# Socrates666/esp32-wake-word

Hardware: AMD Instinct MI355X
Metric: audio windows/sec (1s@16kHz, 40-MFCC) through xiaoa CNN at 1/2/4/8 MI355X (higher is better)
Workload: dtype f32; 1 GPU; config2: fused MFCC(torchaudio+CMVN)+xiaoa CNN fp32, B clips per GPU; audio=fp32 samples, batch_per_gpu=65536, global_batch=65536, seq_len=16000, parallelism=dp1 (per-rank clip split, no collectives), process_group_world_size=1

## Files before the change

### esp32-wake-word_amd/csrc/wk_fe_dev.h

```cpp
#pragma once
#include "wk_common.h"
#include "wk_tables.h"

namespace wk {

__device__ __forceinline__ f2 w32(int k2) {
  switch (k2) {
    case 0: return {1.0f, 0.0f};
    case 1: return {0.98078528040323043f, -0.19509032201612825f};
    case 2: return {0.92387953251128674f, -0.38268343236508978f};
    case 3: return {0.83146961230254524f, -0.55557023301960218f};
    case 4: return {0.70710678118654752f, -0.70710678118654752f};
    case 5: return {0.55557023301960218f, -0.83146961230254524f};
    case 6: return {0.38268343236508978f, -0.92387953251128674f};
    case 7: return {0.19509032201612825f, -0.98078528040323043f};
    default: return {0.0f, -1.0f};
  }
}

template <typename T>
struct Raw {
  T x0[10], x1[10];
  T xb;
};

template <typename T> __device__ __forceinline__ T raw_ld(__amdgpu_buffer_rsrc_t r, int idx);
template <> __device__ __forceinline__ float raw_ld<float>(__amdgpu_buffer_rsrc_t r, int idx) {
  return __builtin_bit_cast(float, __builtin_amdgcn_raw_buffer_load_b32(r, idx * 4, 0, 0));
}
template <> __device__ __forceinline__ int16_t raw_ld<int16_t>(__amdgpu_buffer_rsrc_t r, int idx) {
  return (int16_t)__builtin_amdgcn_raw_buffer_load_b16(r, idx * 2, 0, 0);
}

template <typename T> __device__ __forceinline__ void raw_ld2(__amdgpu_buffer_rsrc_t r, int idx, T& a, T& b);
template <> __device__ __forceinline__ void raw_ld2<float>(__amdgpu_buffer_rsrc_t r, int idx, float& a, float& b) {
  const auto v = __builtin_amdgcn_raw_buffer_load_b64(r, idx * 4, 0, 0);
  a = __uint_as_float(v[0]);
  b = __uint_as_float(v[1]);
}
template <> __device__ __forceinline__ void raw_ld2<int16_t>(__amdgpu_buffer_rsrc_t r, int idx, int16_t& a,
                                                            int16_t& b) {
  const uint32_t v = __builtin_amdgcn_raw_buffer_load_b32(r, idx * 2, 0, 0);
  a = (int16_t)(v & 0xFFFFu);
  b = (int16_t)(v >> 16);
}

__device__ __forceinline__ int refl_idx(int i, int n) {
  i = i < 0 ? -i : i;
  return i > n - 1 ? 2 * (n - 1) - i : i;
}

template <bool MODE_B, typename T>
__device__ __forceinline__ void load_raw(__amdgpu_buffer_rsrc_t rs, int base, int j, int n, bool act, bool general,
                                         Raw<T>& r, int off = 0) {
  if (!act) return;
  if (!general) {
    const int v0 = base + 2 * j;
#pragma unroll
    for (int n1 = 0; n1 < 10; ++n1) raw_ld2<T>(rs, v0 + 32 * n1, r.x0[n1], r.x1[n1]);
    r.xb = raw_ld<T>(rs, base - 1);
  } else {
#pragma unroll
    for (int n1 = 0; n1 < 10; ++n1) {
      const int i0 = base + 32 * n1 + 2 * j;
      r.x0[n1] = raw_ld<T>(rs, off + (MODE_B ? refl_idx(i0, n) : i0));
      r.x1[n1] = raw_ld<T>(rs, off + (MODE_B ? refl_idx(i0 + 1, n) : i0 + 1));
    }
    const int ib = j == 15 ? base + 32 * 9 + 32 : base - 1;
    r.xb = raw_ld<T>(rs, off + (MODE_B ? refl_idx(ib, n) : ib));
  }
}

__device__ __forceinline__ constexpr int pf_part(int n1) {
  return WK_FE_STAGED ? n1 / 3 : (n1 < 4 ? 0 : n1 < 7 ? 1 : n1 < 9 ? 2 : 3);
}
template <bool MODE_B, typename T>
__device__ __forceinline__ void load_raw_part(__amdgpu_buffer_rsrc_t rs, int base, int j, int n, bool act,
                                              bool general, Raw<T>& r, int part) {
  if (!act) return;
  if (general) {
    if (part == 0) load_raw<MODE_B, T>(rs, base, j, n, act, true, r);
    return;
  }
  const int v0 = base + 2 * j;
#pragma unroll
  for (int n1 = 0; n1 < 10; ++n1)
    if (pf_part(n1) == part) raw_ld2<T>(rs, v0 + 32 * n1, r.x0[n1], r.x1[n1]);
  if (part == 0) r.xb = raw_ld<T>(rs, base - 1);
}

struct NoPrefetch {
  __device__ __forceinline__ void operator()(int) const {}
};

__device__ __forceinline__ float row_ror1(float v) {
  return __int_as_float(__builtin_amdgcn_mov_dpp(__float_as_int(v), 0x121, 0xF, 0xF, false));
}
__device__ __forceinline__ float row_rol1(float v) {
  return __int_as_float(__builtin_amdgcn_mov_dpp(__float_as_int(v), 0x12F, 0xF, 0xF, false));
}

struct FeTables {
  const float* win;
  const float* tw;
};

struct TwsLds {
  const float* p;
  __device__ __forceinline__ f2 operator()(int k2, int j) const {
    return *reinterpret_cast<const f2*>(p + ((k2 - 1) * 16 + j) * 2);
  }
};

__device__ __forceinline__ bool fe_split_flip(int j, int k2) {
  return j == 8 || (j >= 1 && j <= 7 && !(k2 & 1)) || (j >= 9 && (k2 & 1));
}
__device__ __forceinline__ f2 fe_split_tw(int j, int k2) {
  float sn, cs;
  sincospif(-(float)(j + 16 * k2) / 256.0f, &sn, &cs);
  return fe_split_flip(j, k2) ? f2{-cs, sn} : f2{cs, sn};
}
__device__ __forceinline__ void fe_init_tws(float* tws, int tid, int nthreads) {
  for (int i = tid; i < 7 * 16; i += nthreads) {
    const f2 w = fe_split_tw(i % 16, i / 16 + 1);
    tws[2 * i] = w.x;
    tws[2 * i + 1] = w.y;
  }
}

template <bool MODE_B, typename T>
__device__ __forceinline__ void fe_stage0(const Raw<T>& raw, int base, int n, int j, bool general,
                                          const FeTables& tb, f2 (&a)[16], float pre = -0.97f WK_SP_PARAM) {
  f2 w[10];
#pragma unroll
  for (int n1 = 0; n1 < 10; ++n1) w[n1] = *reinterpret_cast<const f2*>(tb.win + 32 * n1 + 2 * j);
  float prev_rot = 0.0f;
  float y0[10], y1[10];
#pragma unroll
  for (int n1 = 0; n1 < 10; ++n1) {
    const float x0 = to_f(raw.x0[n1]), x1 = to_f(raw.x1[n1]);
    float rot = row_ror1(x1);
    asm volatile("" : "+v"(rot));
    const float xm = j != 0 ? rot : (n1 == 0 ? to_f(raw.xb) : prev_rot);
    prev_rot = rot;
    y0[n1] = __builtin_fmaf(pre, xm, x0);
    y1[n1] = __builtin_fmaf(pre, x0, x1);
  }
  if (MODE_B && general) {
#pragma unroll
    for (int n1 = 0; n1 < 10; ++n1) {
      const float x0 = to_f(raw.x0[n1]), x1 = to_f(raw.x1[n1]);
      const int i0 = base + 32 * n1 + 2 * j;
      float nx = row_rol1(x0);
      float nx1 = row_rol1(to_f(raw.x0[n1 + 1 < 10 ? n1 + 1 : 9]));
      asm volatile("" : "+v"(nx), "+v"(nx1));
      const float xn = j != 15 ? nx : (n1 < 9 ? nx1 : to_f(raw.xb));
      const bool reflected = i0 < 0 || i0 > n - 1;
      const float r0 = __builtin_fmaf(pre, x1, x0), r1 = __builtin_fmaf(pre, xn, x1);
      const float g0 = reflected ? r0 : (i0 == 0 ? x0 : y0[n1]);
      const float g1 = reflected ? r1 : y1[n1];
      a[n1] = f2{g0, g1} * w[n1];
    }
  } else {
#pragma unroll
    for (int n1 = 0; n1 < 10; ++n1) a[n1] = f2{y0[n1], y1[n1]} * w[n1];
  }
#pragma unroll
  for (int n1 = 10; n1 < 16; ++n1) a[n1] = f2{0.0f, 0.0f};
}

template <bool MODE_B, typename PF, typename TWS>
__device__ __forceinline__ void fe_rest(f2 (&a)[16], int j, float* __restrict__ row, float* __restrict__ xs,
                                        const FeTables& tb, f2 w0, const TWS& tws, int esp_pack,
                                        const PF& pf WK_SP_PARAM) {
  pf(0);
  dft16(a);
  WK_FE_HIT(2);

  f2* x2 = reinterpret_cast<f2*>(xs);
  const int wb = 17 * (j & 7) + (j & 8);
  auto tw = [&](int s) { return cmul2(a[dft16_out(s)], *reinterpret_cast<const f2*>(tb.tw + (s * 16 + j) * 2)); };
  f2 b[8];
  if constexpr (!WK_FE_STAGED) pf(1);
#pragma unroll
  for (int s = 0; s < 8; ++s) b[s] = tw(s);
  pf(-1);
#pragma unroll
  for (int s = 0; s < 8; ++s) x2[wb + s] = b[s];
  WK_FE_HIT(3);
  if constexpr (WK_FE_STAGED) pf(1);
  f2 c[16];
  wave_lds_sync();
#pragma unroll
  for (int s = 0; s < 8; ++s) c[s] = x2[j + 17 * s];
  if constexpr (!WK_FE_STAGED) pf(2);
#pragma unroll
  for (int s = 8; s < 16; ++s) b[s - 8] = tw(s);
  wave_lds_sync();
#pragma unroll
  for (int s = 8; s < 16; ++s) x2[wb + s - 8] = b[s - 8];
  wave_lds_sync();
#pragma unroll
  for (int s = 8; s < 16; ++s) c[s] = x2[(j ^ 8) + 17 * (s - 8)];
  wave_lds_sync();
  WK_FE_HIT(4);

  if constexpr (WK_FE_STAGED) {
    pf(2);
    dft16(c);
    pf(3);
  } else {
    pf(3);
    dft16(c);
  }
  WK_FE_HIT(5);

  f2 sc0 = {1.0f, 1.0f}, sc = {1.0f, 1.0f};
  if constexpr (!MODE_B) {
    const float e = esp_pack ? 4.0f / 2048.0f : 1.0f / 2048.0f;
    sc = f2{e, e};
    sc0 = esp_pack ? (j == 0 ? f2{1.0f / 2048.0f, 0.0f} : sc) : sc;
  }
  {
    const f2 z = c[dft16_out(8)];
    float p128 = 4.0f * __builtin_fmaf(z.x, z.x, z.y * z.y);
    if constexpr (!MODE_B) p128 = __builtin_fmaf(p128, sc.x, 1e-12f);
    if (j == 0) row[128] = p128;
  }
  constexpr int G = 3;
#pragma unroll
  for (int k0 = 0; k0 < 8; k0 += G) {
    f2 S[G], D[G], pw[G];
#if WK_FE_STAGED
    float mx[G], my[G];
#pragma unroll
    for (int t = 0; t < G; ++t)
      if (k0 + t <= 7) {
        const f2 sv = c[dft16_out(15 - k0 - t)];
        mx[t] = dpp<0x140>(sv.x);
        my[t] = dpp<0x140>(sv.y);
      }
#pragma unroll
    for (int t = 0; t < G; ++t) {
      const int k2 = k0 + t;
      if (k2 > 7) continue;
      const f2 zk = c[dft16_out(k2)];
      const f2 own = c[dft16_out((16 - k2) & 15)];
      f2 zq;
      zq.x = __int_as_float(__builtin_amdgcn_update_dpp(__float_as_int(own.x), __float_as_int(mx[t]), 0x111, 0xF, 0xF, false));
      zq.y = __int_as_float(__builtin_amdgcn_update_dpp(__float_as_int(own.y), __float_as_int(my[t]), 0x111, 0xF, 0xF, false));
      S[t] = fma2(zq, f2{1.0f, -1.0f}, zk);
      D[t] = fma2(zq, f2{-1.0f, 1.0f}, zk);
    }
#else
#pragma unroll
    for (int t = 0; t < G; ++t) {
      const int k2 = k0 + t;
      if (k2 > 7) continue;
      const f2 zk = c[dft16_out(k2)];
      const f2 sv = c[dft16_out(15 - k2)];
      const f2 own = c[dft16_out((16 - k2) & 15)];
      f2 zq;
      zq.x = __int_as_float(__builtin_amdgcn_update_dpp(__float_as_int(own.x), __float_as_int(dpp<0x140>(sv.x)),
                                                        0x111, 0xF, 0xF, false));
      zq.y = __int_as_float(__builtin_amdgcn_update_dpp(__float_as_int(own.y), __float_as_int(dpp<0x140>(sv.y)),
                                                        0x111, 0xF, 0xF, false));
      S[t] = fma2(zq, f2{1.0f, -1.0f}, zk);
      D[t] = fma2(zq, f2{-1.0f, 1.0f}, zk);
    }
#endif
#if WK_FE_STAGED
    f2 wt[G], tt[G], bb[G], uvx[G], uvy[G], sq[G];
#pragma unroll
    for (int t = 0; t < G; ++t)
      if (k0 + t <= 7) {
        wt[t] = k0 + t == 0 ? w0 : tws(k0 + t, j);
        tt[t] = cmul2_a(D[t], wt[t]);
      }
#pragma unroll
    for (int t = 0; t < G; ++t)
      if (k0 + t <= 7) bb[t] = cmul2_b(D[t], wt[t], tt[t]);
#pragma unroll
    for (int t = 0; t < G; ++t)
      if (k0 + t <= 7) {
        uvx[t] = fma2(by(bb[t]), f2{1.0f, -1.0f}, bx(S[t]));
        uvy[t] = fma2(bx(bb[t]), f2{-1.0f, 1.0f}, by(S[t]));
      }
#pragma unroll
    for (int t = 0; t < G; ++t)
      if (k0 + t <= 7) sq[t] = uvy[t] * uvy[t];
#pragma unroll
    for (int t = 0; t < G; ++t) {
      const int k2 = k0 + t;
      if (k2 > 7) continue;
      pw[t] = fma2(uvx[t], uvx[t], sq[t]);
      if constexpr (!MODE_B) pw[t] = fma2(pw[t], k2 == 0 ? sc0 : sc, f2{1e-12f, 1e-12f});
    }
#else
#pragma unroll
    for (int t = 0; t < G; ++t) {
      const int k2 = k0 + t;
      if (k2 > 7) continue;
      const f2 bb = cmul2(D[t], k2 == 0 ? w0 : tws(k2, j));
      const f2 uvx = fma2(by(bb), f2{1.0f, -1.0f}, bx(S[t]));
      const f2 uvy = fma2(bx(bb), f2{-1.0f, 1.0f}, by(S[t]));
      pw[t] = fma2(uvx, uvx, uvy * uvy);
      if constexpr (!MODE_B) pw[t] = fma2(pw[t], k2 == 0 ? sc0 : sc, f2{1e-12f, 1e-12f});
    }
#endif
#pragma unroll
    for (int t = 0; t < G; ++t)
      if (k0 + t <= 7) row[j + 16 * (k0 + t)] = pw[t].x;
#pragma unroll
    for (int t = 0; t < G; ++t)
      if (k0 + t <= 7) row[256 - j - 16 * (k0 + t)] = pw[t].y;
  }
  WK_FE_HIT(6);
}

template <bool MODE_B, int W>
__device__ __forceinline__ void mel_wave(const float* p, float* l) {
  if constexpr (MODE_B) melB_wave<W>(p, l); else melA_wave<W>(p, l);
}

template <bool MODE_B>
__device__ __forceinline__ void mel_dispatch(int wave, const float* p, float* l) {
  switch (wave) {
    case 0: mel_wave<MODE_B, 0>(p, l); break;
    case 1: mel_wave<MODE_B, 1>(p, l); break;
    case 2: mel_wave<MODE_B, 2>(p, l); break;
    case 3: mel_wave<MODE_B, 3>(p, l); break;
    case 4: mel_wave<MODE_B, 4>(p, l); break;
    case 5: mel_wave<MODE_B, 5>(p, l); break;
    case 6: mel_wave<MODE_B, 6>(p, l); break;
    default: mel_wave<MODE_B, 7>(p, l); break;
  }
}

__device__ __forceinline__ float cmvn_lane(float v, bool valid, int n) {
  const float mean = wave_sum(valid ? v : 0.0f) / (float)n;
  const float d = valid ? v - mean : 0.0f;
  float sd = sqrtf(wave_sum(d * d) / (float)(n - 1));
  sd = sd == 0.0f ? 1.0f : sd;
  return d * (1.0f / (sd + 1e-8f));
}

__device__ __forceinline__ void cmvn_lane2(float& v0, float& v1, bool valid, int n) {
  const float m0 = wave_sum(valid ? v0 : 0.0f) / (float)n;
  const float m1 = wave_sum(valid ? v1 : 0.0f) / (float)n;
  const float d0 = valid ? v0 - m0 : 0.0f;
  const float d1 = valid ? v1 - m1 : 0.0f;
  float s0 = sqrtf(wave_sum(d0 * d0) / (float)(n - 1));
  float s1 = sqrtf(wave_sum(d1 * d1) / (float)(n - 1));
  s0 = s0 == 0.0f ? 1.0f : s0;
  s1 = s1 == 0.0f ? 1.0f : s1;
  v0 = d0 * (1.0f / (s0 + 1e-8f));
  v1 = d1 * (1.0f / (s1 + 1e-8f));
}

constexpr int kTwOff = 0, kTwSize = 16 * 16 * 2;
constexpr int kTwsOff = kTwOff + kTwSize, kTwsSize = 7 * 16 * 2;
constexpr int kLOff = kTwsOff + kTwsSize, kLSize = 40 * WK_LSTRIDE;
constexpr int kPOff = kLOff + kLSize, kPSize = kNFramesB * kPRow;
constexpr int kFeLdsNoWin = kPOff + kPSize;
constexpr int kWinOff = (kFeLdsNoWin + 1) & ~1, kWinSize = 320;
constexpr int kFeLds = kWinOff + kWinSize;
static_assert(kFeLdsNoWin * 4 <= 81920, "standalone front-end LDS must allow 2 workgroups per CU");
static_assert(kLOff % 4 == 0, "log-mel rows are read with ds_read_b128");
static_assert(kPOff % 2 == 0 && kPRow % 2 == 1 && kPRow >= 271,
              "row f's transpose scratch is row + (f & 1): 8-byte aligned, 270 floats");

template <bool MODE_B, bool WIN>
__device__ __forceinline__ void fe_init_tables(float* smem, int tid, int nthreads) {
  if (WIN)
    for (int i = tid; i < 320; i += nthreads) smem[kWinOff + i] = MODE_B ? kWinB[i] : kWinA[i];
  for (int i = tid; i < 16 * 16; i += nthreads) {
    const int s = i / 16, jj = i % 16, k1 = s ^ (jj & 8);
    float sn, cs;
    sincospif(-(float)(jj * k1) / 128.0f, &sn, &cs);
    smem[kTwOff + 2 * i] = cs;
    smem[kTwOff + 2 * i + 1] = sn;
  }
  fe_init_tws(smem + kTwsOff, tid, nthreads);
}

}
```

### esp32-wake-word_amd/csrc/wk_fused.hip

```cpp
#define WK_FUSED_TU
#include "wk_cnn_dev.h"
#include "wk_fe_dev.h"
#include "wk_kernels.h"

using namespace wk;

#if !(defined(WK_FUSED_XDL_TU) && WK_FUSED_ONE_TU)
namespace {

#ifdef WK_DIAG
__device__ unsigned long long g_wk_stamps[16][16];
#define WK_STAMP_INIT WkStamps _stamps; _stamps.init();
#define WK_STAMP(k) _stamps.hit(k)
#define WK_STAMP_FLUSH(w) do { if (lane == 0) for (int _k = 0; _k < 16; ++_k) atomicAdd(&g_wk_stamps[w][_k], _stamps.st[_k]); } while (0)
#define WK_SP_ARG , &_stamps
#else
#define WK_STAMP_INIT
#define WK_STAMP(k) do {} while (0)
#define WK_STAMP_FLUSH(w) do {} while (0)
#define WK_SP_ARG
#endif



constexpr int NBF = 4;
#ifndef WK_FE_WAVES
#define WK_FE_WAVES 8
#endif
#if WK_FE_WAVES != 8 && !defined(WK_DIAG)
#error "WK_FE_WAVES != 8 is a diagnostic build (front-end role alone, WAKEWORD_FUSED_EXP=1)"
#endif
constexpr int kFeWaves = WK_FE_WAVES;
constexpr int kFusedBlock = 1024;
constexpr int kGOff = (kFeLds + 3) & ~3;
constexpr int kFcpOff = kGOff + 128 * NBF;
constexpr int kFcpSize = 8 * NBF * 64;
constexpr int kL1Off = kFcpOff + kFcpSize;
static_assert(kLOff % 4 == 0 && kL1Off % 4 == 0, "log-mel buffers are read with ds_read_b128");
constexpr int kCtrlOff = kL1Off + kLSize;
constexpr int kImgOff = (kCtrlOff + 16 + 3) & ~3;
constexpr int I0_CIP = 24, I1_CIP = 40, I2_CIP = 72;
constexpr int I0_TP = 64, I1_TP = 32, I2_TP = 18;
constexpr int F0_CIP = 20, F1_CIP = 36, F2_CIP = 68;
constexpr int kF0Off = kImgOff;
constexpr int kF1Off = kF0Off + NBF * I0_TP * F0_CIP;
constexpr int kF2Off = kF1Off + NBF * I1_TP * F1_CIP;
constexpr int kF2End = kF2Off + NBF * I2_TP * F2_CIP;
constexpr int kImgEnd = kImgOff + NBF * (I0_TP * 40 + I1_TP * 72 + I2_TP * 136) / 2 > kF2End
                            ? kImgOff + NBF * (I0_TP * 40 + I1_TP * 72 + I2_TP * 136) / 2
                            : kF2End;
constexpr int kB0Off = kImgOff;
constexpr int kB1Off = kB0Off + NBF * I0_TP * I0_CIP / 2;
constexpr int kB2Off = kB1Off + NBF * I1_TP * I1_CIP / 2;
constexpr int X0_CIP = 40, X1_CIP = 72, X2_CIP = 136;
constexpr int kX0Off = kImgOff;
constexpr int kX1Off = kX0Off + NBF * I0_TP * X0_CIP / 2;
constexpr int kX2Off = kX1Off + NBF * I1_TP * X1_CIP / 2;
static_assert(kX2Off + NBF * I2_TP * X2_CIP / 2 <= kImgEnd, "split images fit the fp32 carve");
static_assert(kF1Off % 4 == 0 && kF2Off % 4 == 0 && kB1Off % 2 == 0 && kB2Off % 2 == 0 && kX1Off % 2 == 0 &&
                  kX2Off % 2 == 0, "vector-aligned images");
enum { kConvF32 = 0, kConvBf16 = 1, kConvBf16x3 = 2 };
constexpr int kDummyRowOff = (kImgEnd + 1) & ~1;
constexpr int kFusedLds = kDummyRowOff + kPRow + 1;
static_assert(kFusedLds * 4 <= 163840, "fused LDS budget");
static_assert(kPOff + kPSize <= kGOff && kLOff + kLSize <= kPOff && kImgEnd <= kDummyRowOff,
              "CNN carve disjoint from the front-end's power rows, log-mel buffer and dummy row");
static_assert(kGOff + 128 * NBF <= kFcpOff && kFcpOff + kFcpSize <= kL1Off && kL1Off + kLSize <= kCtrlOff &&
                  kCtrlOff + 16 <= kImgOff,
              "pooled features | partials | log-mel buffer 1 | control words, in that order, disjoint");
static_assert(kF2End <= kImgEnd && kB2Off + NBF * I2_TP * I2_CIP / 2 <= kImgEnd &&
                  kX2Off + NBF * I2_TP * X2_CIP / 2 <= kImgEnd,
              "every precision's conv images end inside [kImgOff, kImgEnd)");

enum { kCtrlFeBar = 0, kCtrlCnnBar = 1, kCtrlLReady = 2, kCtrlLFree = 4, kCtrlAbort = 15 };
static_assert(kCtrlOff % 4 == 0 && kCtrlLFree % 4 == 0, "spin_until_all8 reads the eight LFree words as two uint4");
constexpr unsigned kSpinLimit = 1u << 22;

__device__ __forceinline__ unsigned lds_load(const unsigned* p) {
  return __hip_atomic_load(p, __ATOMIC_RELAXED, __HIP_MEMORY_SCOPE_WORKGROUP);
}
__device__ __forceinline__ unsigned lds_load_u(const unsigned* p) {
  return __builtin_amdgcn_readfirstlane(lds_load(p));
}

constexpr int kPrioFe = 3;
constexpr int kSpinSleep = 2;

template <int PRIO, typename F>
__device__ __forceinline__ void spin_on(unsigned* ctrl, const F& ready) {
  __atomic_signal_fence(__ATOMIC_SEQ_CST);
  if (!ready()) {
    if (PRIO > 0) __builtin_amdgcn_s_setprio(0);
    for (unsigned n = 4;; n += 4) {
      __builtin_amdgcn_s_sleep(kSpinSleep);
      if (ready()) break;
      __builtin_amdgcn_s_sleep(kSpinSleep);
      if (ready()) break;
      __builtin_amdgcn_s_sleep(kSpinSleep);
      if (ready()) break;
      __builtin_amdgcn_s_sleep(kSpinSleep);
      if (ready()) break;
      if ((n & 31) == 0 && (n >= kSpinLimit || lds_load_u(ctrl + kCtrlAbort))) {
        __hip_atomic_store(ctrl + kCtrlAbort, 1u, __ATOMIC_RELAXED, __HIP_MEMORY_SCOPE_WORKGROUP);
        break;
      }
    }
    if (PRIO > 0) __builtin_amdgcn_s_setprio(PRIO);
  }
  asm volatile("" ::: "memory");
  __atomic_signal_fence(__ATOMIC_SEQ_CST);
}

template <int PRIO>
__device__ __forceinline__ void spin_until(unsigned* ctrl, int idx, unsigned v) {
  spin_on<PRIO>(ctrl, [=] { return lds_load_u(ctrl + idx) >= v; });
}

template <int PRIO, int N = 8>
__device__ __forceinline__ void role_sync(unsigned* ctrl, int idx, unsigned& gen, int lane) {
  gen += N;
  __atomic_signal_fence(__ATOMIC_SEQ_CST);
  asm volatile("s_waitcnt lgkmcnt(0)" ::: "memory");
  if (lane == 0) __hip_atomic_fetch_add(ctrl + idx, 1u, __ATOMIC_RELAXED, __HIP_MEMORY_SCOPE_WORKGROUP);
  spin_until<PRIO>(ctrl, idx, gen);
}

__device__ __forceinline__ unsigned min8(const unsigned* ctrl, int idx) {
  asm volatile("" ::: "memory");
  const uint4* q = reinterpret_cast<const uint4*>(ctrl + idx);
  const uint4 a = q[0], b = q[1];
  return min(min(min(a.x, a.y), min(a.z, a.w)), min(min(b.x, b.y), min(b.z, b.w)));
}
template <int PRIO>
__device__ __forceinline__ void spin_until_all8(unsigned* ctrl, int idx, unsigned v) {
  spin_on<PRIO>(ctrl, [=] { return __builtin_amdgcn_readfirstlane(min8(ctrl, idx)) >= v; });
}

__device__ __forceinline__ void signal_set(unsigned* ctrl, int idx, unsigned v, int lane) {
  __atomic_signal_fence(__ATOMIC_SEQ_CST);
  asm volatile("s_waitcnt lgkmcnt(0)" ::: "memory");
  if (lane == 0) __hip_atomic_store(ctrl + idx, v, __ATOMIC_RELAXED, __HIP_MEMORY_SCOPE_WORKGROUP);
  __atomic_signal_fence(__ATOMIC_SEQ_CST);
}

__device__ __forceinline__ void signal_add(unsigned* ctrl, int idx, int lane) {
  __atomic_signal_fence(__ATOMIC_SEQ_CST);
  asm volatile("s_waitcnt lgkmcnt(0)" ::: "memory");
  if (lane == 0) __hip_atomic_fetch_add(ctrl + idx, 1u, __ATOMIC_RELAXED, __HIP_MEMORY_SCOPE_WORKGROUP);
  __atomic_signal_fence(__ATOMIC_SEQ_CST);
}

template <typename T, int FEW = 8>
__device__ __forceinline__ void fe_role(float* smem, const T* __restrict__ audio, int64_t n_mine,
                                        int64_t clip_stride, float* __restrict__ feats_out, int wave, int lane,
                                        int diag) {
  static_assert(FEW == 8 || FEW == 12, "8 or 12 front-end waves");
  float* P = smem + kPOff;
  float* L = smem + kLOff;
  float* L1 = smem + kL1Off;
  unsigned* ctrl = reinterpret_cast<unsigned*>(smem + kCtrlOff);
  const int g = lane >> 4, j = lane & 15;
  const FeTables tb = {smem + kWinOff, smem + kTwOff};
  const TwsLds tws = {smem + kTwsOff};
  const f2 w0 = fe_split_tw(j, 0);
  const int slot_base = 16 * (g & 1) + 32 * (g >> 1);
  const int fw = FEW == 8 || wave < 8 ? wave : wave - 4;
  const int r0 = FEW == 8 || wave < 8 ? 0 : 1, r1 = FEW == 8 || wave < 4 ? 1 : r0;
  const bool mel_wave = FEW == 8 || wave >= 4;
  const int melw = FEW == 8 ? wave : wave - 4;
  const int64_t G = gridDim.x;
  unsigned gen = 0, p_wait = 0;

  const int64_t step = G * clip_stride;
  const T* cptr = audio + (int64_t)blockIdx.x * clip_stride;
  constexpr uint32_t kClipBytes = kWinSamples * sizeof(T);
  struct PfCtx {
    __amdgpu_buffer_rsrc_t rs;
    int base;
    bool general;
  };
  auto fwr = [&](int r) { return FEW == 8 && WK_FE_STAGED && r == 1 ? fw ^ 4 : fw; };
  auto pf_ctx = [&](const T* p, bool ok, int r) -> PfCtx {
    const int fl = fwr(r) + 8 * r + slot_base;
    return {make_rsrc(p, ok ? kClipBytes : 0u), 256 * fl - 160, (r == 0 && fwr(r) == 0) || (r == 1 && fwr(r) == 6)};
  };

  Raw<T> pf;
  {
    const PfCtx c0 = pf_ctx(cptr, n_mine > 0, r0);
    load_raw<true>(c0.rs, c0.base, j, kWinSamples, true, c0.general, pf);
  }
  WK_STAMP_INIT
  for (int64_t i = 0; i < n_mine; ++i) {
#pragma unroll 1
    for (int r = r0; r <= r1; ++r) {
      const int fl = fwr(r) + 8 * r + slot_base;
      const bool general = (r == 0 && fwr(r) == 0) || (r == 1 && fwr(r) == 6);
      f2 a[16];
#ifdef WK_DIAG
      asm volatile("s_waitcnt vmcnt(0)" ::: "memory");
      WK_STAMP(11);
#endif
      fe_stage0<true>(pf, 256 * fl - 160, kWinSamples, j, general, tb, a);
      WK_STAMP(0);
      const PfCtx nx = r < r1 ? pf_ctx(cptr, true, r + 1) : pf_ctx(cptr + step, i + 1 < n_mine, r0);
      auto pf_part = [&](int k) {
        if (k >= 0) {
          load_raw_part<true>(nx.rs, nx.base, j, kWinSamples, true, nx.general, pf, k);
        } else if (r == r0) {
          spin_until<kPrioFe>(ctrl, kCtrlFeBar, p_wait);
          WK_STAMP(9);
        }
      };
      WK_STAMP(1);
      float* row = fl < kNFramesB ? P + fl * kPRow : smem + kDummyRowOff;
      fe_rest<true>(a, j, row, row + (fl & 1), tb, w0, tws, 0, pf_part WK_SP_ARG);
    }
    role_sync<kPrioFe, FEW>(ctrl, kCtrlFeBar, gen, lane);
    WK_STAMP(7);
    if (mel_wave && i >= 2 && !(diag & 1)) spin_until_all8<kPrioFe>(ctrl, kCtrlLFree, (unsigned)(i - 1));
    WK_STAMP(10);
    if (mel_wave) {
      int prow = kPOff + min(lane, kNFramesB - 1) * kPRow;
      asm volatile("" : "+v"(prow));
      mel_dispatch<true>(melw, smem + prow, (i & 1 ? L1 : L) + lane);
      WK_STAMP(8);
      signal_add(ctrl, kCtrlLReady, lane);
    }
    gen += FEW;
    signal_add(ctrl, kCtrlFeBar, lane);
    p_wait = gen;
    cptr += step;
  }
  WK_STAMP_FLUSH(wave);
}

__device__ __forceinline__ float row_sum16(float v) {
  v += dpp<0xB1>(v);
  v += dpp<0x4E>(v);
  v += dpp<0x141>(v);
  v += dpp<0x140>(v);
  return v;
}

template <int CM>
__device__ __forceinline__ void dct_cmvn_clip(const float* __restrict__ lbuf, int slot, float* __restrict__ F0,
                                              uint16_t* __restrict__ B0, uint16_t* __restrict__ X0,
                                              float* __restrict__ fo, int lane) {
  const int li = lane & 15, lk = lane >> 4;
  int aoff = 4 * (li * 40 + lk);
  asm volatile("" : "+v"(aoff));
  const auto ra = make_rsrc(kDctB16, sizeof(kDctB16));
  float dA[10];
#pragma unroll
  for (int s = 0; s < 10; ++s) dA[s] = buf_load(ra, aoff, 16 * s);
  f32x4 d[4] = {{0, 0, 0, 0}, {0, 0, 0, 0}, {0, 0, 0, 0}, {0, 0, 0, 0}};
#pragma unroll
  for (int s = 0; s < 10; ++s) {
    const f32x4 b = *reinterpret_cast<const f32x4*>(lbuf + (4 * s + lk) * WK_LSTRIDE + 4 * li);
#pragma unroll
    for (int nt = 0; nt < 4; ++nt) d[nt] = mfma4(dA[s], b[nt], d[nt]);
  }
  const bool v3 = li != 15;
  float mean[4], inv[4];
#pragma unroll
  for (int r = 0; r < 4; ++r) {
    const float x3 = v3 ? d[3][r] : 0.0f;
    mean[r] = row_sum16((d[0][r] + d[1][r]) + (d[2][r] + x3)) * (1.0f / kNFramesB);
    float dv[4];
#pragma unroll
    for (int nt = 0; nt < 4; ++nt) dv[nt] = d[nt][r] - mean[r];
    dv[3] = v3 ? dv[3] : 0.0f;
    const float q = row_sum16((dv[0] * dv[0] + dv[1] * dv[1]) + (dv[2] * dv[2] + dv[3] * dv[3]));
    float sd = __builtin_amdgcn_sqrtf(q * (1.0f / (kNFramesB - 1)));
    sd = sd == 0.0f ? 1.0f : sd;
    inv[r] = __builtin_amdgcn_rcpf(sd + 1e-8f);
  }
#pragma unroll
  for (int nt = 0; nt < 4; ++nt) {
    const int t = 4 * li + nt;
    if (nt == 3 && !v3) continue;
    const int row = slot * I0_TP + 1 + t;
    float y[4];
#pragma unroll
    for (int r = 0; r < 4; ++r) y[r] = (d[nt][r] - mean[r]) * inv[r];
    if constexpr (CM == kConvBf16) {
      uint2 pk;
      pk.x = bf16_bits(y[0]) | (bf16_bits(y[1]) << 16);
      pk.y = bf16_bits(y[2]) | (bf16_bits(y[3]) << 16);
      *reinterpret_cast<uint2*>(B0 + row * I0_CIP + 4 * lk) = pk;
    } else if constexpr (CM == kConvBf16x3) {
      uint32_t h[4], l[4];
#pragma unroll
      for (int r = 0; r < 4; ++r) {
        h[r] = bf16_bits(y[r]);
        l[r] = bf16_bits(y[r] - __uint_as_float(h[r] << 16));
      }
      *reinterpret_cast<uint2*>(X0 + row * X0_CIP + 4 * lk) = make_uint2(h[0] | (h[1] << 16), h[2] | (h[3] << 16));
      *reinterpret_cast<uint2*>(X0 + row * X0_CIP + 16 + 4 * lk) = make_uint2(l[0] | (l[1] << 16), l[2] | (l[3] << 16));
    } else {
      *reinterpret_cast<f32x4*>(F0 + row * F0_CIP + 4 * lk) = f32x4{y[0], y[1], y[2], y[3]};
    }
    if (fo) {
#pragma unroll
      for (int r = 0; r < 4; ++r)
        if (4 * lk + r < 13) fo[(4 * lk + r) * kNFramesB + t] = y[r];
    }
  }
}

template <int CM, class SRC>
__device__ __forceinline__ void cnn_role(float* base, const float* __restrict__ pk, const uint16_t* __restrict__ pkb,
                                         int64_t n_mine, int64_t clip_base, int64_t clip_step,
                                         float* __restrict__ logits, int cw, int lane, SRC& src) {
  float* F0 = base + kF0Off;
  float* F1 = base + kF1Off;
  float* F2 = base + kF2Off;
  uint16_t* B0 = reinterpret_cast<uint16_t*>(base + kB0Off);
  uint16_t* B1 = reinterpret_cast<uint16_t*>(base + kB1Off);
  uint16_t* B2 = reinterpret_cast<uint16_t*>(base + kB2Off);
  uint16_t* X0 = reinterpret_cast<uint16_t*>(base + kX0Off);
  uint16_t* X1 = reinterpret_cast<uint16_t*>(base + kX1Off);
  uint16_t* X2 = reinterpret_cast<uint16_t*>(base + kX2Off);
  constexpr bool BF = CM == kConvBf16, X3 = CM == kConvBf16x3;
  constexpr int kLoW = kNumPackedBf16;
  const auto rsb = make_rsrc(pkb, 2 * kNumPackedBf16 * (X3 ? 2 : 1));
  auto frag_bf = [&](int elem_off) -> s8 {
    return __builtin_bit_cast(s8, __builtin_amdgcn_raw_buffer_load_b128(rsb, 16 * lane, 2 * elem_off, 0));
  };
  float* Gp = base + kGOff;
  float* FCP = base + kFcpOff;
  unsigned* ctrl = reinterpret_cast<unsigned*>(base + kCtrlOff);
  const int li = lane & 15, lk = lane >> 4;
  unsigned gen = 0;
  const auto rs = make_rsrc(pk, 4 * kNumPacked);
  const int lv = 4 * lane;

  float w3[48];
  s8 w3b[6];
  if constexpr (BF || X3) {
#pragma unroll
    for (int s = 0; s < 6; ++s) w3b[s] = frag_bf(kPbW3 + (cw * 6 + s) * kBfFrag);
  }
  if constexpr (CM == kConvF32) {
#pragma unroll
    for (int s = 0; s < 48; ++s) w3[s] = buf_load(rs, lv, 4 * (kPkW3 + (cw * 48 + s) * 64));
  }
  const int64_t n_batches = (n_mine + NBF - 1) / NBF;
  src.init(cw, lane);
  bool eager_done = false;
  auto try_eager = [&](int64_t b) {
    if (cw >= NBF || eager_done) return;
    const int64_t i = (b + 1) * NBF + cw;
    if (i >= n_mine) return;
    if (src.ready(i)) {
      src.load(i, cw);
      eager_done = true;
    }
  };
  auto fc2 = [&](int64_t bb) {
    if (cw != 0) return;
    int ln = lane;
    asm volatile("" : "+v"(ln));
    const int cl = ln & (NBF - 1), q = ln >> 2;
    float h[4];
    if constexpr (CM == kConvF32) {
      f32x4 v = *reinterpret_cast<const f32x4*>(FCP + cl * 64 + 4 * q);
#pragma unroll
      for (int w = 1; w < 8; ++w) v += *reinterpret_cast<const f32x4*>(FCP + (w * NBF + cl) * 64 + 4 * q);
#pragma unroll
      for (int r = 0; r < 4; ++r) h[r] = v[r];
    } else {
      const f32x4 v = *reinterpret_cast<const f32x4*>(FCP + cl * 64 + 4 * q);
#pragma unroll
      for (int r = 0; r < 4; ++r) h[r] = v[r];
#pragma unroll
      for (int w = 1; w < 8; ++w) {
        const f32x4 u = *reinterpret_cast<const f32x4*>(FCP + (w * NBF + cl) * 64 + 4 * q);
#pragma unroll
        for (int r = 0; r < 4; ++r) h[r] += u[r];
      }
    }
    float acc = 0.0f;
#pragma unroll
    for (int i2 = 0; i2 < 4; ++i2) acc = __builtin_fmaf(buf_load(rs, 16 * q, 4 * (kPkF2 + i2)), fmaxf(h[i2], 0.0f), acc);
    acc += __shfl_xor(acc, 4, 64);
    acc += __shfl_xor(acc, 8, 64);
    acc += __shfl_xor(acc, 16, 64);
    acc += __shfl_xor(acc, 32, 64);
    const int64_t i = bb * NBF + cl;
    if (q == 0 && i < n_mine) logits[clip_base + clip_step * i] = acc;
  };
  WK_STAMP_INIT
  for (int64_t b = 0; b < n_batches; ++b) {
    if (cw < NBF && !eager_done) {
      const int64_t i = b * NBF + cw;
      if (i < n_mine) {
        src.wait(i);
        src.load(i, cw);
      }
    }
    eager_done = false;
    float w1[12];
    s8 w1b[2], w1l[2];
    if constexpr (BF || X3) {
#pragma unroll
      for (int s = 0; s < 2; ++s) w1b[s] = frag_bf(kPbW1 + ((cw & 1) * 2 + s) * kBfFrag);
    }
    if constexpr (X3) {
#pragma unroll
      for (int s = 0; s < 2; ++s) w1l[s] = frag_bf(kLoW + kPbW1 + ((cw & 1) * 2 + s) * kBfFrag);
    }
    if constexpr (CM == kConvF32) {
#pragma unroll
      for (int s = 0; s < 12; ++s) w1[s] = buf_load(rs, lv, 4 * (kPkW1 + ((cw & 1) * 12 + s) * 64));
    }
    WK_STAMP(0);
    role_sync<0>(ctrl, kCtrlCnnBar, gen, lane);
    if (b > 0) fc2(b - 1);

    const int nv = n_mine - b * NBF < NBF ? (int)(n_mine - b * NBF) : NBF;

    if ((cw >> 1) < nv) {
      const int co0 = 16 * (cw & 1), cl = cw >> 1;
      const int bo = (cl * I0_TP + li) * I0_CIP;
#pragma unroll 1
      for (int p = 0; p < 2; ++p) {
        const int ta = 32 * p, tb = ta + 16;
        f32x4 acc_a = {0, 0, 0, 0}, acc_b = {0, 0, 0, 0};
        if constexpr (BF) {
          conv_pair_bf<2, 16, I0_CIP>(B0, w1b, bo + ta * I0_CIP, bo + tb * I0_CIP, lk, acc_a, acc_b);
          epi_pool_bf<I1_CIP, I1_TP, 31>(acc_a, B1, co0, cl, ta, lane);
          epi_pool_bf<I1_CIP, I1_TP, 31>(acc_b, B1, co0, cl, tb, lane);
        } else if constexpr (X3) {
          const int bx = (cl * I0_TP + li) * X0_CIP;
          conv_pair_bf3<2, 16, X0_CIP>(X0, w1b, w1l, bx + ta * X0_CIP, bx + tb * X0_CIP, lk, acc_a, acc_b);
          epi_pool_bf3<X1_CIP, I1_TP, 31, 32>(acc_a, X1, co0, cl, ta, lane);
          epi_pool_bf3<X1_CIP, I1_TP, 31, 32>(acc_b, X1, co0, cl, tb, lane);
        } else {
          f32x4 m[4] = {{0, 0, 0, 0}, {0, 0, 0, 0}, {0, 0, 0, 0}, {0, 0, 0, 0}};
          conv_wino_v<1, F0_CIP>(F0, w1, (cl * I0_TP + 2 * (16 * p + li)) * F0_CIP + 4 * lk, m);
          epi_wino_pool<F1_CIP, I1_TP, 31>(m, F1, co0, cl, 16 * p, lane);
        }
      }
    }
    WK_STAMP(1);
    role_sync<0>(ctrl, kCtrlCnnBar, gen, lane);
    try_eager(b);
    WK_STAMP(2);

    if constexpr (BF) {
      s8 w2b[3];
#pragma unroll
      for (int s = 0; s < 3; ++s) w2b[s] = frag_bf(kPbW2 + ((cw & 3) * 3 + s) * kBfFrag);
      const int co0 = 16 * (cw & 3);
#pragma unroll 1
      for (int p = 0; p < 2; ++p) {
        const int cl = 2 * (cw >> 2) + p;
        if (cl >= nv) break;
        const int bb = (cl * I1_TP + li) * I1_CIP;
        f32x4 acc_a = {0, 0, 0, 0}, acc_b = {0, 0, 0, 0};
        conv_pair_bf<3, 32, I1_CIP>(B1, w2b, bb, bb + 16 * I1_CIP, lk, acc_a, acc_b);
        epi_pool_bf<I2_CIP, I2_TP, 15>(acc_a, B2, co0, cl, 0, lane);
        epi_pool_bf<I2_CIP, I2_TP, 15>(acc_b, B2, co0, cl, 16, lane);
      }
    } else if constexpr (X3) {
      s8 w2b[3], w2l[3];
#pragma unroll
      for (int s = 0; s < 3; ++s) w2b[s] = frag_bf(kPbW2 + ((cw & 3) * 3 + s) * kBfFrag);
#pragma unroll
      for (int s = 0; s < 3; ++s) w2l[s] = frag_bf(kLoW + kPbW2 + ((cw & 3) * 3 + s) * kBfFrag);
      const int co0 = 16 * (cw & 3);
#pragma unroll 1
      for (int p = 0; p < 2; ++p) {
        const int cl = 2 * (cw >> 2) + p;
        if (cl >= nv) break;
        const int bb = (cl * I1_TP + li) * X1_CIP;
        f32x4 acc_a = {0, 0, 0, 0}, acc_b = {0, 0, 0, 0};
        conv_pair_bf3<3, 32, X1_CIP>(X1, w2b, w2l, bb, bb + 16 * X1_CIP, lk, acc_a, acc_b);
        epi_pool_bf3<X2_CIP, I2_TP, 15, 64>(acc_a, X2, co0, cl, 0, lane);
        epi_pool_bf3<X2_CIP, I2_TP, 15, 64>(acc_b, X2, co0, cl, 16, lane);
      }
    } else {
      float w2[24];
#pragma unroll
      for (int s = 0; s < 24; ++s) w2[s] = buf_load(rs, lv, 4 * (kPkW2 + ((cw & 3) * 24 + s) * 64));
      const int co0 = 16 * (cw & 3);
#pragma unroll 1
      for (int p = 0; p < 2; ++p) {
        const int cl = 2 * (cw >> 2) + p;
        if (cl >= nv) break;
        f32x4 m[4] = {{0, 0, 0, 0}, {0, 0, 0, 0}, {0, 0, 0, 0}, {0, 0, 0, 0}};
        conv_wino_v<2, F1_CIP, 1>(F1, w2, (cl * I1_TP + 2 * li) * F1_CIP + 4 * lk, m);
        epi_wino_pool<F2_CIP, I2_TP, 15>(m, F2, co0, cl, 0, lane);
      }
    }
    WK_STAMP(3);
    role_sync<0>(ctrl, kCtrlCnnBar, gen, lane);
    try_eager(b);
    WK_STAMP(4);

    {
      const int co0 = 16 * cw;
      const int bo = li * I2_CIP;
#pragma unroll 1
      for (int p = 0; p < 2; ++p) {
        if (p > 0) try_eager(b);
        const int ca = 2 * p, cb = 2 * p + 1;
        if (ca >= nv) break;
        f32x4 acc_a = {0, 0, 0, 0}, acc_b = {0, 0, 0, 0};
        if constexpr (BF) {
          conv_pair_bf<6, 64, I2_CIP, 3>(B2, w3b, bo + ca * I2_TP * I2_CIP, bo + cb * I2_TP * I2_CIP, lk, acc_a,
                                         acc_b);
        } else if constexpr (X3) {
          s8 w3l[6];
#pragma unroll
          for (int s = 0; s < 6; ++s) w3l[s] = frag_bf(kLoW + kPbW3 + (cw * 6 + s) * kBfFrag);
          const int bx = li * X2_CIP;
          conv_pair_bf3<6, 64, X2_CIP, 2>(X2, w3b, w3l, bx + ca * I2_TP * X2_CIP, bx + cb * I2_TP * X2_CIP, lk,
                                          acc_a, acc_b);
        } else {
          f32x4 m[4] = {{0, 0, 0, 0}, {0, 0, 0, 0}, {0, 0, 0, 0}, {0, 0, 0, 0}};
          conv_wino_v<4, F2_CIP, 1>(F2, w3, ((ca + (li >> 3)) * I2_TP + 2 * (li & 7)) * F2_CIP + 4 * lk, m);
          epi_wino_gap<NBF>(m, Gp, co0, ca, lane);
          continue;
        }
        epi_gap<NBF>(acc_a, Gp, co0, ca, lane);
        epi_gap<NBF>(acc_b, Gp, co0, cb, lane);
      }
    }
    float wf1[16];
    {
#pragma unroll
      for (int s = 0; s < 16; ++s) wf1[s] = buf_load(rs, lv, 4 * (kPkF1 + (cw * 16 + s) * 64));
    }
    WK_STAMP(5);
    role_sync<0>(ctrl, kCtrlCnnBar, gen, lane);
    try_eager(b);
    WK_STAMP(6);

    {
      int ln = lane;
      asm volatile("" : "+v"(ln));
      f32x4 acc = {0, 0, 0, 0};
      const float* g = Gp + 16 * cw * NBF + (ln & (NBF - 1));
#pragma unroll
      for (int s = 0; s < 16; ++s) acc = mfma4x4(wf1[s], g[s * NBF], acc);
      *reinterpret_cast<f32x4*>(FCP + (cw * NBF + (ln & (NBF - 1))) * 64 + 4 * (ln >> 2)) = acc;
    }
    try_eager(b);
    WK_STAMP(8);
  }
  if (n_batches > 0) {
    role_sync<0>(ctrl, kCtrlCnnBar, gen, lane);
    fc2(n_batches - 1);
  }
  WK_STAMP_FLUSH(8 + cw);
}

template <int CM, bool FEATS>
struct LogmelSrc {
  float* smem;
  unsigned* ctrl;
  float* feats_out;
  int64_t clip_base, clip_step;
  int cw, lane, diag;
  __device__ __forceinline__ void init(int cw_, int lane_) {
    cw = cw_;
    lane = lane_;
    signal_set(ctrl, kCtrlLFree + cw, cw < NBF ? (unsigned)cw : 0xFFFFFFFFu, lane);
  }
  __device__ __forceinline__ bool ready(int64_t i) const {
    __atomic_signal_fence(__ATOMIC_SEQ_CST);
    const bool r = (diag & 2) ||
                   __builtin_amdgcn_readfirstlane(lds_load(ctrl + kCtrlLReady)) >= 8u * (unsigned)(i + 1);
    asm volatile("" ::: "memory");
    __atomic_signal_fence(__ATOMIC_SEQ_CST);
    return r;
  }
  __device__ __forceinline__ void wait(int64_t i) const {
    if (!(diag & 2)) spin_until<0>(ctrl, kCtrlLReady, 8u * (unsigned)(i + 1));
  }
  __device__ __forceinline__ void load(int64_t i, int slot) const {
    float* fo = FEATS ? feats_out + (clip_base + clip_step * i) * (13 * kNFramesB) : nullptr;
    dct_cmvn_clip<CM>(smem + (i & 1 ? kL1Off : kLOff), slot, smem + kF0Off,
                      reinterpret_cast<uint16_t*>(smem + kB0Off), reinterpret_cast<uint16_t*>(smem + kX0Off), fo,
                      lane);
    signal_set(ctrl, kCtrlLFree + cw, (unsigned)(i + NBF), lane);
  }
};

__device__ __forceinline__ void report_abort(const unsigned* ctrl, unsigned* err, int lane) {
  if (lane == 0 && err) {
    const unsigned ab = lds_load(ctrl + kCtrlAbort);
    if (ab) __hip_atomic_store(err, ab == 1u ? 1u : 3u, __ATOMIC_RELAXED, __HIP_MEMORY_SCOPE_SYSTEM);
  }
}

template <typename T, int CM, bool FEATS>
__global__ __launch_bounds__(kFusedBlock, 4) void wk_fused_kernel(const T* __restrict__ audio, int64_t batch,
                                                                 int64_t clip_stride, const float* __restrict__ wts,
                                                                 const uint16_t* __restrict__ wbf,
                                                                 float* __restrict__ logits,
                                                                 float* __restrict__ feats_out, unsigned* err,
                                                                 int diag) {
  __shared__ __attribute__((aligned(16))) float smem[kFusedLds];
#ifndef WK_DIAG
  diag = 0;
#endif
  const int tid = threadIdx.x;
  const int lane = tid & 63;
  const int wave = __builtin_amdgcn_readfirstlane(tid >> 6);
  fe_init_tables<true, true>(smem, tid, kFusedBlock);
  for (int i = tid; i < kFusedLds - kGOff; i += kFusedBlock) smem[kGOff + i] = 0.0f;
  __syncthreads();
  const int64_t n_mine = batch > (int64_t)blockIdx.x ? (batch - 1 - blockIdx.x) / gridDim.x + 1 : 0;
  if (wave < kFeWaves) __builtin_amdgcn_s_setprio(kPrioFe);
  if (wave < kFeWaves) {
    if (!(diag & 2)) fe_role<T, kFeWaves>(smem, audio, n_mine, clip_stride, feats_out, wave, lane, diag);
  } else {
    if (!(diag & 1)) {
      LogmelSrc<CM, FEATS> src = {smem, reinterpret_cast<unsigned*>(smem + kCtrlOff), feats_out, (int64_t)blockIdx.x,
                                  (int64_t)gridDim.x, 0, 0, diag};
      cnn_role<CM>(smem, wts, wbf, n_mine, (int64_t)blockIdx.x, (int64_t)gridDim.x, logits, wave - 8, lane, src);
    }
  }
  report_abort(reinterpret_cast<unsigned*>(smem + kCtrlOff), err, lane);
}

template <int CM>
struct FeatSrc {
  const float* feats;
  float* base;
  int64_t clip_base, clip_step;
  int lane;
  __device__ __forceinline__ void init(int, int lane_) { lane = lane_; }
  __device__ __forceinline__ bool ready(int64_t) const { return true; }
  __device__ __forceinline__ void wait(int64_t) const {}
  __device__ __forceinline__ void load(int64_t i, int slot) const {
    const float* f = feats + (clip_base + clip_step * i) * (13 * kNFramesB);
    if (lane >= kNFramesB) return;
    float y[13];
#pragma unroll
    for (int c = 0; c < 13; ++c) y[c] = __builtin_nontemporal_load(f + c * kNFramesB + lane);
    const int row = slot * I0_TP + 1 + lane;
    if constexpr (CM == kConvBf16) {
      uint16_t* B0 = reinterpret_cast<uint16_t*>(base + kB0Off) + row * I0_CIP;
#pragma unroll
      for (int c = 0; c < 12; c += 4)
        *reinterpret_cast<uint2*>(B0 + c) = make_uint2(bf16_bits(y[c]) | (bf16_bits(y[c + 1]) << 16),
                                                       bf16_bits(y[c + 2]) | (bf16_bits(y[c + 3]) << 16));
      B0[12] = (uint16_t)bf16_bits(y[12]);
    } else if constexpr (CM == kConvBf16x3) {
      uint16_t* X0 = reinterpret_cast<uint16_t*>(base + kX0Off) + row * X0_CIP;
#pragma unroll
      for (int c = 0; c < 13; ++c) {
        const uint32_t h = bf16_bits(y[c]);
        X0[c] = (uint16_t)h;
        X0[16 + c] = (uint16_t)bf16_bits(y[c] - __uint_as_float(h << 16));
      }
    } else {
      float* F0 = base + kF0Off + row * F0_CIP;
#pragma unroll
      for (int c = 0; c < 12; c += 4) *reinterpret_cast<f32x4*>(F0 + c) = f32x4{y[c], y[c + 1], y[c + 2], y[c + 3]};
      F0[12] = y[12];
    }
  }
};

constexpr int kCnnCarve = kImgEnd - kGOff;
constexpr int kCnnLds = 2 * kCnnCarve;
static_assert(kCnnLds * 4 <= 163840, "standalone CNN LDS budget");
static_assert(kCnnCarve % 4 == 0 && kGOff % 4 == 0, "16-byte aligned carves");

template <int CM>
__global__ __launch_bounds__(kFusedBlock, 4) void wk_cnn_fused_kernel(const float* __restrict__ feats, int64_t batch,
                                                                     const float* __restrict__ wts,
                                                                     const uint16_t* __restrict__ wbf,
                                                                     float* __restrict__ logits, unsigned* err) {
  __shared__ __attribute__((aligned(16))) float smem[kCnnLds];
  const int tid = threadIdx.x, lane = tid & 63;
  const int wave = __builtin_amdgcn_readfirstlane(tid >> 6);
  for (int i = tid; i < kCnnLds; i += kFusedBlock) smem[i] = 0.0f;
  __syncthreads();
  const int role = wave >> 3;
  float* base = smem + role * kCnnCarve - kGOff;
  const int64_t cb = 2 * (int64_t)blockIdx.x + role, cs = 2 * (int64_t)gridDim.x;
  const int64_t n_mine = batch > cb ? (batch - 1 - cb) / cs + 1 : 0;
  FeatSrc<CM> src = {feats, base, cb, cs, 0};
  cnn_role<CM>(base, wts, wbf, n_mine, cb, cs, logits, wave & 7, lane, src);
  report_abort(reinterpret_cast<const unsigned*>(base + kCtrlOff), err, lane);
}

}

#ifndef WK_FUSED_XDL_TU
#ifdef WK_DIAG
extern "C" int wk_debug_stamps(unsigned long long* host_out, int reset) {
  if (hipMemcpyFromSymbol(host_out, HIP_SYMBOL(g_wk_stamps), sizeof(g_wk_stamps)) != hipSuccess) return 1;
  if (reset) {
    static unsigned long long zero[16][16];
    if (hipMemcpyToSymbol(HIP_SYMBOL(g_wk_stamps), zero, sizeof(zero)) != hipSuccess) return 1;
  }
  return 0;
}
#endif

#endif

namespace wk {

#ifdef WK_FUSED_XDL_TU
hipError_t launch_fused_xdl(bool i16, const void* audio, int64_t batch, int64_t clip_stride, const float* w,
                            const uint16_t* wbf, int conv_mode, float* logits, float* feats_or_null, int grid_cap,
                            hipStream_t stream, unsigned* err, int diag) {
#else
hipError_t launch_fused(bool i16, const void* audio, int64_t batch, int64_t clip_stride, const float* w,
                        const uint16_t* wbf, int conv_mode, float* logits, float* feats_or_null, int grid_cap,
                        hipStream_t stream, unsigned* err, int diag) {
#endif
  if (batch == 0) return hipSuccess;
  const int grid = (int)(batch < grid_cap ? batch : grid_cap);
  const dim3 g(grid), blk(kFusedBlock);
  if (conv_mode != kConvF32 && !wbf) return hipErrorInvalidValue;
#if !WK_FUSED_ONE_TU && !defined(WK_FUSED_XDL_TU)
  if (conv_mode != kConvF32)
    return launch_fused_xdl(i16, audio, batch, clip_stride, w, wbf, conv_mode, logits, feats_or_null, grid_cap, stream,
                            err, diag);
#endif
#define WK_FUSED_LAUNCH(T, CM)                                                                              \
  do {                                                                                                         \
    if (feats_or_null)                                                                                         \
      hipLaunchKernelGGL((wk_fused_kernel<T, CM, true>), g, blk, 0, stream, (const T*)audio, batch, clip_stride, \
                         w, wbf, logits, feats_or_null, err, diag);                                               \
    else                                                                                                       \
      hipLaunchKernelGGL((wk_fused_kernel<T, CM, false>), g, blk, 0, stream, (const T*)audio, batch,            \
                         clip_stride, w, wbf, logits, nullptr, err, diag);                                        \
  } while (0)
#if defined(WK_FUSED_XDL_TU)
  if (i16) {
    if (conv_mode == kConvBf16x3) WK_FUSED_LAUNCH(int16_t, kConvBf16x3);
    else WK_FUSED_LAUNCH(int16_t, kConvBf16);
  } else {
    if (conv_mode == kConvBf16x3) WK_FUSED_LAUNCH(float, kConvBf16x3);
    else WK_FUSED_LAUNCH(float, kConvBf16);
  }
#elif !WK_FUSED_ONE_TU
  if (i16) WK_FUSED_LAUNCH(int16_t, kConvF32);
  else WK_FUSED_LAUNCH(float, kConvF32);
#else
  if (i16) {
    if (conv_mode == kConvBf16) WK_FUSED_LAUNCH(int16_t, kConvBf16);
    else if (conv_mode == kConvBf16x3) WK_FUSED_LAUNCH(int16_t, kConvBf16x3);
    else WK_FUSED_LAUNCH(int16_t, kConvF32);
  } else {
    if (conv_mode == kConvBf16) WK_FUSED_LAUNCH(float, kConvBf16);
    else if (conv_mode == kConvBf16x3) WK_FUSED_LAUNCH(float, kConvBf16x3);
    else WK_FUSED_LAUNCH(float, kConvF32);
  }
#endif
#undef WK_FUSED_LAUNCH
  return hipGetLastError();
}

#ifndef WK_FUSED_XDL_TU

hipError_t launch_cnn_fused(const float* feats, int64_t batch, const float* w, const uint16_t* wbf, int conv_mode,
                            float* logits, int grid_cap, hipStream_t stream, unsigned* err) {
  if (batch == 0) return hipSuccess;
  if (conv_mode != kConvF32 && !wbf) return hipErrorInvalidValue;
  const int64_t roles = (batch + NBF - 1) / NBF;
  const int grid = (int)((roles + 1) / 2 < grid_cap ? (roles + 1) / 2 : grid_cap);
  if (conv_mode == kConvBf16)
    hipLaunchKernelGGL(wk_cnn_fused_kernel<kConvBf16>, dim3(grid), dim3(kFusedBlock), 0, stream, feats, batch, w, wbf,
                       logits, err);
  else if (conv_mode == kConvBf16x3)
    hipLaunchKernelGGL(wk_cnn_fused_kernel<kConvBf16x3>, dim3(grid), dim3(kFusedBlock), 0, stream, feats, batch, w,
                       wbf, logits, err);
  else
    hipLaunchKernelGGL(wk_cnn_fused_kernel<kConvF32>, dim3(grid), dim3(kFusedBlock), 0, stream, feats, batch, w, wbf,
                       logits, err);
  return hipGetLastError();
}
#endif

}
#endif
```

Baseline: 35.00 million windows/s.

## Handle reflect-padding edges with DPP lane shuffles instead of scalar general loads

Replaces the 'general' path for reflect-padded edge frames, which issued per-element scalar loads with reflected indices, with the same vectorized paired loads used for interior frames. Reflection and pre-emphasis at the edge frames are then rebuilt in registers using DPP row mirror/shift operations. This makes prefetch uniform, so edge waves no longer do all loads in part 0, and removes divergent scalar loads from the edge waves. It also adds a macro to decouple the round-1 wave swap from the staged mode. The cost is more intricate lane-shuffle logic, which risks correctness bugs at the boundaries.

```diff
diff --git a/esp32-wake-word_amd/csrc/wk_fe_dev.h b/esp32-wake-word_amd/csrc/wk_fe_dev.h
--- a/esp32-wake-word_amd/csrc/wk_fe_dev.h
+++ b/esp32-wake-word_amd/csrc/wk_fe_dev.h
@@ -74,19 +74,14 @@
 __device__ __forceinline__ constexpr int pf_part(int n1) {
   return WK_FE_STAGED ? n1 / 3 : (n1 < 4 ? 0 : n1 < 7 ? 1 : n1 < 9 ? 2 : 3);
 }
-template <bool MODE_B, typename T>
-__device__ __forceinline__ void load_raw_part(__amdgpu_buffer_rsrc_t rs, int base, int j, int n, bool act,
-                                              bool general, Raw<T>& r, int part) {
-  if (!act) return;
-  if (general) {
-    if (part == 0) load_raw<MODE_B, T>(rs, base, j, n, act, true, r);
-    return;
-  }
+template <typename T>
+__device__ __forceinline__ void load_raw_part(__amdgpu_buffer_rsrc_t rs, int base, int xb_idx, int j, Raw<T>& r,
+                                              int part) {
   const int v0 = base + 2 * j;
 #pragma unroll
   for (int n1 = 0; n1 < 10; ++n1)
     if (pf_part(n1) == part) raw_ld2<T>(rs, v0 + 32 * n1, r.x0[n1], r.x1[n1]);
-  if (part == 0) r.xb = raw_ld<T>(rs, base - 1);
+  if (part == 0) r.xb = raw_ld<T>(rs, xb_idx);
 }
 
 struct NoPrefetch {
@@ -165,6 +160,65 @@
 #pragma unroll
     for (int n1 = 0; n1 < 10; ++n1) a[n1] = f2{y0[n1], y1[n1]} * w[n1];
   }
+#pragma unroll
+  for (int n1 = 10; n1 < 16; ++n1) a[n1] = f2{0.0f, 0.0f};
+}
+
+template <int CTRL, int ROWS>
+__device__ __forceinline__ float dpp_rows(float old, float src) {
+  return __int_as_float(__builtin_amdgcn_update_dpp(__float_as_int(old), __float_as_int(src), CTRL, ROWS, 0xF, false));
+}
+template <int EDGE, typename T>
+__device__ __forceinline__ void fe_stage0_rows(const Raw<T>& raw, int lane, const f2 (&w)[10], f2 (&a)[16],
+                                               float pre) {
+  const int j = lane & 15;
+  float prev_rot = 0.0f;
+#pragma unroll
+  for (int n1 = 0; n1 < 10; ++n1) {
+    const float x0 = to_f(raw.x0[n1]), x1 = to_f(raw.x1[n1]);
+    float rot = row_ror1(x1);
+    asm volatile("" : "+v"(rot));
+    const float xm = j != 0 ? rot : (n1 == 0 ? to_f(raw.xb) : prev_rot);
+    prev_rot = rot;
+    float c0 = x0, c1 = x1, pm = xm, p1 = x0;
+    if constexpr (EDGE == 1) {
+      if (n1 < 5) {
+        const float m0 = to_f(raw.x0[9 - n1]), m1 = to_f(raw.x1[9 - n1]);
+        p1 = dpp_rows<0x140, 0x1>(x0, m0);
+        c1 = dpp_rows<0x140, 0x1>(x1, m1);
+        pm = dpp_rows<0x140, 0x1>(xm, m1);
+        asm volatile("" : "+v"(p1), "+v"(c1), "+v"(pm));
+        const float l0 = n1 == 0 ? to_f(raw.xb) : to_f(raw.x0[10 - n1]);
+        c0 = dpp_rows<0x111, 0x1>(lane == 0 ? l0 : x0, p1);
+        asm volatile("" : "+v"(c0));
+      }
+    } else if constexpr (EDGE == 2) {
+      if (n1 == 9) {
+        const float q0 = to_f(raw.x0[8]), q1 = to_f(raw.x1[8]);
+        c0 = dpp_rows<0x140, 0x8>(x0, q0);
+        float s1 = dpp_rows<0x140, 0x8>(x1, q1);
+        asm volatile("" : "+v"(c0), "+v"(s1));
+        p1 = dpp_rows<0x101, 0x8>(lane == 63 ? to_f(raw.x0[7]) : x0, c0);
+        c1 = dpp_rows<0x101, 0x8>(lane == 63 ? to_f(raw.x1[7]) : x1, s1);
+        asm volatile("" : "+v"(p1), "+v"(c1));
+        pm = lane >= 48 ? c1 : xm;
+      }
+    }
+    float y0 = __builtin_fmaf(pre, pm, c0);
+    const float y1 = __builtin_fmaf(pre, p1, c1);
+    if (EDGE == 1 && n1 == 5) y0 = lane == 0 ? x0 : y0;
+    a[n1] = f2{y0, y1} * w[n1];
+  }
+}
+template <typename T>
+__device__ __forceinline__ void fe_stage0_fused(const Raw<T>& raw, int lane, int edge, const FeTables& tb,
+                                                f2 (&a)[16], float pre = -0.97f) {
+  f2 w[10];
+#pragma unroll
+  for (int n1 = 0; n1 < 10; ++n1) w[n1] = *reinterpret_cast<const f2*>(tb.win + 32 * n1 + 2 * (lane & 15));
+  if (edge == 0) fe_stage0_rows<0>(raw, lane, w, a, pre);
+  else if (edge == 1) fe_stage0_rows<1>(raw, lane, w, a, pre);
+  else fe_stage0_rows<2>(raw, lane, w, a, pre);
 #pragma unroll
   for (int n1 = 10; n1 < 16; ++n1) a[n1] = f2{0.0f, 0.0f};
 }
diff --git a/esp32-wake-word_amd/csrc/wk_fused.hip b/esp32-wake-word_amd/csrc/wk_fused.hip
--- a/esp32-wake-word_amd/csrc/wk_fused.hip
+++ b/esp32-wake-word_amd/csrc/wk_fused.hip
@@ -31,6 +31,9 @@
 #error "WK_FE_WAVES != 8 is a diagnostic build (front-end role alone, WAKEWORD_FUSED_EXP=1)"
 #endif
 constexpr int kFeWaves = WK_FE_WAVES;
+#ifndef WK_FE_ROUND1_SWAP
+#define WK_FE_ROUND1_SWAP WK_FE_STAGED
+#endif
 constexpr int kFusedBlock = 1024;
 constexpr int kGOff = (kFeLds + 3) & ~3;
 constexpr int kFcpOff = kGOff + 128 * NBF;
@@ -177,36 +180,37 @@
   struct PfCtx {
     __amdgpu_buffer_rsrc_t rs;
     int base;
-    bool general;
+    int xb;
   };
-  auto fwr = [&](int r) { return FEW == 8 && WK_FE_STAGED && r == 1 ? fw ^ 4 : fw; };
+  auto fwr = [&](int r) { return FEW == 8 && WK_FE_ROUND1_SWAP && r == 1 ? fw ^ 4 : fw; };
   auto pf_ctx = [&](const T* p, bool ok, int r) -> PfCtx {
     const int fl = fwr(r) + 8 * r + slot_base;
-    return {make_rsrc(p, ok ? kClipBytes : 0u), 256 * fl - 160, (r == 0 && fwr(r) == 0) || (r == 1 && fwr(r) == 6)};
+    return {make_rsrc(p, ok ? kClipBytes : 0u), 256 * fl - 160, fl == 0 ? 160 : 256 * fl - 161};
   };
 
   Raw<T> pf;
   {
     const PfCtx c0 = pf_ctx(cptr, n_mine > 0, r0);
-    load_raw<true>(c0.rs, c0.base, j, kWinSamples, true, c0.general, pf);
+#pragma unroll
+    for (int k = 0; k < 4; ++k) load_raw_part(c0.rs, c0.base, c0.xb, j, pf, k);
   }
   WK_STAMP_INIT
   for (int64_t i = 0; i < n_mine; ++i) {
 #pragma unroll 1
     for (int r = r0; r <= r1; ++r) {
       const int fl = fwr(r) + 8 * r + slot_base;
-      const bool general = (r == 0 && fwr(r) == 0) || (r == 1 && fwr(r) == 6);
+      const int edge = r == 0 && fwr(r) == 0 ? 1 : r == 1 && fwr(r) == 6 ? 2 : 0;
       f2 a[16];
 #ifdef WK_DIAG
       asm volatile("s_waitcnt vmcnt(0)" ::: "memory");
       WK_STAMP(11);
 #endif
-      fe_stage0<true>(pf, 256 * fl - 160, kWinSamples, j, general, tb, a);
+      fe_stage0_fused(pf, lane, edge, tb, a);
       WK_STAMP(0);
       const PfCtx nx = r < r1 ? pf_ctx(cptr, true, r + 1) : pf_ctx(cptr + step, i + 1 < n_mine, r0);
       auto pf_part = [&](int k) {
         if (k >= 0) {
-          load_raw_part<true>(nx.rs, nx.base, j, kWinSamples, true, nx.general, pf, k);
+          load_raw_part(nx.rs, nx.base, nx.xb, j, pf, k);
         } else if (r == r0) {
           spin_until<kPrioFe>(ctrl, kCtrlFeBar, p_wait);
           WK_STAMP(9);
```

Measured after the change: 35.99 million windows/s, median of 6. +2.8%, better.
